# mstebelev/wormhole

Hardware: AMD Instinct MI355X
Metric: examples/sec, DiFacto FM on Criteo-1TB-shaped sparse at 1/2/4/8 MI355X (higher is better)
Workload: dtype fp32; 1 GPU; model=difacto-fm-dim64, global_batch=100000, seq_len=39, parallelism=dp1+kvshard1, minibatch_per_gpu=100000, threshold=100, nnz_per_example=39

## Files before the change

csrc/bind/fm_ops.cc:

```cpp
#include "kv_store.h"
#include "localize_ahead.h"
#include "ps_ops.h"
#include "store_guard.h"

#include <c10/hip/HIPCachingAllocator.h>
#include <c10/hip/HIPGuard.h>

#include <cmath>
#include <cstring>
#include <memory>

#include "host/linear_guard_plan.h"

namespace wh_bind {
namespace {

void check_vstride(int64_t vstride) {
  TORCH_CHECK(vstride == 0 || (vstride >= 4 && vstride <= 256 && (vstride & (vstride - 1)) == 0),
              "vstride must be 0 or 4 * 2^k <= 256, got ", vstride);
}

int loss_flags(int64_t loss, const Tensor& met) {
  return (int)loss | (met.numel() >= 5 ? 256 : 0);
}
// ... 580 lines not shown
 private:
  KVStore* store_;
  std::vector<double> hp_;
  int64_t threshold_;
  bool l1_shrk_;
  int64_t seed_, loss_;
  int vs_ = 0;
  double clip_ = 0, dropout_ = 0;
  bool gnorm_ = false, post_on_ = false, direct_ = false, fused_v_ = false;
  int64_t dim_ = 0;
  StoreGuard guard_;
  LocalizeAhead ahead_;
  std::unique_ptr<HostSplit> timing_{host_split("difacto native step")};
};

}

void bind_fm(py::module_& m) {
  py::class_<LinearStep>(m, "LinearStep")
      .def(py::init<KVStore*, int64_t, double, double, double, double, int64_t, double, bool>(),
           py::arg("store"), py::arg("algo"), py::arg("alpha"), py::arg("beta"), py::arg("l1"),
           py::arg("l2"), py::arg("loss"), py::arg("max_load") = 0.7, py::arg("direct") = true,
           py::keep_alive<1, 2>())
      .def("step", &LinearStep::step, py::arg("keys"), py::arg("offset"), py::arg("val"),
           py::arg("label"), py::arg("train"), py::arg("met"), py::arg("auc_sum"),
           py::arg("next_keys") = py::none(), py::arg("next_offset") = py::none(),
           py::arg("next_val") = py::none(), py::arg("ready") = 0)
      .def("reset", &LinearStep::reset)
      .def("guard_sync", &LinearStep::guard_sync)
      .def_property_readonly("grows", &LinearStep::grows)
      .def_property_readonly("direct", [](const LinearStep& l) { return l.direct(); })
      .def_property("pushes", &LinearStep::pushes, &LinearStep::set_pushes);
  py::class_<DifactoStep>(m, "DifactoStep")
      .def(py::init<KVStore*, std::vector<double>, int64_t, bool, int64_t, int64_t,
                    std::vector<double>, double, bool, bool>(),
           py::arg("store"), py::arg("hp"), py::arg("threshold"), py::arg("l1_shrk"),
           py::arg("seed"), py::arg("loss"), py::arg("post"), py::arg("max_load"),
           py::arg("direct"), py::arg("fused_v") = true, py::keep_alive<1, 2>())
      .def("step", &DifactoStep::step, py::arg("keys"), py::arg("offset"), py::arg("val"),
           py::arg("label"), py::arg("train"), py::arg("data_pass"), py::arg("met"),
           py::arg("auc_sum"), py::arg("step"), py::arg("next_keys") = py::none(),
           py::arg("next_offset") = py::none(), py::arg("next_val") = py::none(),
           py::arg("ready") = 0)
      .def("reset", &DifactoStep::reset)
      .def("guard_sync", &DifactoStep::guard_sync)
      .def_property_readonly("direct", &DifactoStep::direct)
      .def_property_readonly("fused_v", &DifactoStep::fused_v)
      .def_property_readonly("grows", &DifactoStep::grows)
      .def_property_readonly("vgrows", &DifactoStep::vgrows);
  m.def("fm_forward", &fm_forward);
  m.def("set_cu_reserve", [](int64_t n) { wh::fm_set_cu_reserve((int)n); },
        "CUs the persistent FM kernels leave free for concurrent collectives");
  m.def("cu_reserve", []() { return (int64_t)wh::fm_cu_reserve(); });
  m.def("fm_backward", &fm_backward);
  m.def("fm_backward_plan", &fm_backward_plan, py::arg("csc_off"), py::arg("csc_row"),
        py::arg("hdr"), py::arg("vc_rows"), py::arg("nrows"), py::arg("vstride"),
        py::arg("two_pass") = false);
  m.def("fm_backward_run", &fm_backward_run);
  m.def("difacto_open_pull_plan", &difacto_open_pull_plan, py::arg("store"), py::arg("keys"),
        py::arg("insert"), py::arg("cnt"), py::arg("h"), py::arg("threshold"),
        py::arg("l1_shrk"), py::arg("seed"), py::arg("direct"), py::arg("csc_off"),
        py::arg("csc_row"), py::arg("nrows"),
        "(tests) the open with the backward's chunk plan: (slot, hdr, vc, vpos, plan)");
  m.def("fm_backward_plan_totals", &fm_backward_plan_totals, py::arg("plan"),
        py::arg("csc_off"), py::arg("nnz"), py::arg("vstride"),
        "(tests) a backward plan's chunk totals {scalar, V}");
  m.def("fm_grad_post", &fm_grad_post);
  m.def("vstride_for", &vstride_for);
  m.def("spmv_t", &spmv_t, py::arg("csc_off"), py::arg("csc_row"), py::arg("csc_val"),
        py::arg("p"));
}

}
```

csrc/hip/fm.hip:

```cpp
#include "wh_common.h"
#include <string>
#include "kv_device.h"
#include "wh_chunk_plan.h"
#include "wh_kernels.h"
#include "wh_lookback.h"
#include "wh_loss.h"

#include <algorithm>
#include <cstdlib>
#include <type_traits>

namespace wh {
namespace {

constexpr int kThreads = 256;
constexpr int kFwdBlocks = 2048;

template <int G>
struct Shape {
  static constexpr int SUB = 64 / G;
  static constexpr int NI = G;
#ifndef WH_FM_TI
#define WH_FM_TI 4
#endif
// ... 214 lines not shown
  if (k < nuniq) {
    vid = key_vidx(hdr, k);
    const int64_t* off = vid >= 0 ? off_v : off_s;
    c0 = off[k];
    nc = (int32_t)(off[k + 1] - c0);
    b0 = (int32_t)csc_off[k];
    cnt = (int32_t)(csc_off[k + 1] - b0);
  }
  emit_key(out, (int32_t)k, c0, nc, b0, cnt, vid, vid >= 0);
}

constexpr int kPlanPer = 4;
constexpr int kPlanTile = kThreads * kPlanPer;

__global__ __launch_bounds__(kThreads) void k_chunk_plan(int64_t nuniq,
                                                         const int64_t* __restrict__ csc_off,
                                                         const float2* __restrict__ hdr,
                                                         Lookback lb, int ntiles,
                                                         int64_t* off_s_tot, int64_t* off_v_tot,
                                                         ChunkOut out) {
  __shared__ uint32_t shs[16];
  __shared__ int sht;
  const int tile = lb_tile(lb, ntiles, &sht);
  const int64_t k0 = (int64_t)tile * kPlanTile + threadIdx.x * kPlanPer;
  int64_t co[kPlanPer + 1];
#pragma unroll
  for (int r = 0; r <= kPlanPer; ++r) co[r] = k0 + r <= nuniq ? csc_off[k0 + r] : 0;
  int32_t vid[kPlanPer];
#pragma unroll
  for (int r = 0; r < kPlanPer; ++r) vid[r] = k0 + r < nuniq ? key_vidx(hdr, k0 + r) : -1;
  uint32_t c[2] = {0u, 0u};
  uint32_t nc[kPlanPer];
#pragma unroll
  for (int r = 0; r < kPlanPer; ++r) {
    nc[r] = k0 + r < nuniq ? (uint32_t)key_chunks(co[r + 1] - co[r], vid[r] >= 0) : 0u;
    c[vid[r] >= 0 ? 1 : 0] += nc[r];
  }
  uint32_t ex[2], tot[2];
  lb_block_scan<2>(lb, tile, c, ex, tot, shs);
  if (tile == ntiles - 1 && threadIdx.x == 0) {
    *off_s_tot = tot[0];
    *off_v_tot = tot[1];
  }
#pragma unroll
  for (int r = 0; r < kPlanPer; ++r) {
    const int isv = vid[r] >= 0;
    emit_key(out, (int32_t)(k0 + r), isv ? ex[1] : ex[0], (int32_t)nc[r], (int32_t)co[r],
             (int32_t)(co[r + 1] - co[r]), vid[r], isv);
    ex[isv ? 1 : 0] += nc[r];
  }
}

constexpr int kBuckets = 256;
constexpr int kBucketBlocks = 128;
constexpr int kBucketU = 8;

__device__ __forceinline__ int row_bucket(int row, int shift) {
  const int b = row >> shift;
  return b < kBuckets ? b : kBuckets - 1;
}

__global__ __launch_bounds__(kThreads) void k_vchunk_hist(const int64_t* __restrict__ nchunk_p,
                                                          const int4* __restrict__ meta,
                                                          const int32_t* __restrict__ csc_row,
                                                          int shift, int32_t* hist) {
  __shared__ int32_t h[kBuckets];
  for (int i = threadIdx.x; i < kBuckets; i += kThreads) h[i] = 0;
  __syncthreads();
  const int64_t n = *nchunk_p;
  const int64_t per = (n + gridDim.x - 1) / gridDim.x;
  const int64_t c0 = per * blockIdx.x, c1 = c0 + per < n ? c0 + per : n;
  for (int64_t cb = c0 + threadIdx.x; cb < c1; cb += kThreads * kBucketU) {
    int idx[kBucketU], row[kBucketU];
#pragma unroll
    for (int u = 0; u < kBucketU; ++u) {
      const int64_t c = cb + (int64_t)u * kThreads;
      idx[u] = c < c1 ? meta[c].y : -1;
    }
#pragma unroll
    for (int u = 0; u < kBucketU; ++u) row[u] = idx[u] >= 0 ? csc_row[idx[u]] : -1;
#pragma unroll
    for (int u = 0; u < kBucketU; ++u)
      if (row[u] >= 0) atomicAdd(&h[row_bucket(row[u], shift)], 1);
  }
  __syncthreads();
  for (int i = threadIdx.x; i < kBuckets; i += kThreads) hist[blockIdx.x * kBuckets + i] = h[i];
}

constexpr int kScanParts = 4;
constexpr int kScanPer = kBucketBlocks / kScanParts;

__global__ __launch_bounds__(kBuckets * kScanParts) void k_vchunk_scan(int32_t* hist) {
  __shared__ int32_t part[kScanParts][kBuckets];
  __shared__ int32_t excl[kBuckets];
  __shared__ int32_t wtot[kBuckets / 64];
  const int b = threadIdx.x & (kBuckets - 1), q = threadIdx.x / kBuckets;
  int32_t v[kScanPer];
#pragma unroll
  for (int i = 0; i < kScanPer; ++i) v[i] = hist[(q * kScanPer + i) * kBuckets + b];
  int32_t sum = 0;
#pragma unroll
  for (int i = 0; i < kScanPer; ++i) sum += v[i];
  part[q][b] = sum;
  __syncthreads();
  if (q == 0) {
    int32_t t = 0;
#pragma unroll
    for (int r = 0; r < kScanParts; ++r) t += part[r][b];
    const int lane = b & 63;
    int32_t x = t;
#pragma unroll
    for (int o = 1; o < 64; o <<= 1) {
      const int32_t y = __shfl_up(x, o, 64);
      if (lane >= o) x += y;
    }
    if (lane == 63) wtot[b >> 6] = x;
    excl[b] = x - t;
  }
  __syncthreads();
  int32_t base = excl[b];
  for (int w = 0; w < (b >> 6); ++w) base += wtot[w];
  for (int r = 0; r < q; ++r) base += part[r][b];
#pragma unroll
  for (int i = 0; i < kScanPer; ++i) {
    hist[(q * kScanPer + i) * kBuckets + b] = base;
    base += v[i];
  }
}

__global__ __launch_bounds__(kThreads) void k_vchunk_scatter(const int64_t* __restrict__ nchunk_p,
                                                             const int4* __restrict__ meta,
                                                             const int32_t* __restrict__ csc_row,
                                                             int shift,
                                                             const int32_t* __restrict__ hist,
                                                             int4* out) {
  __shared__ int32_t base[kBuckets];
  for (int i = threadIdx.x; i < kBuckets; i += kThreads) base[i] = hist[blockIdx.x * kBuckets + i];
  __syncthreads();
  const int64_t n = *nchunk_p;
  const int64_t per = (n + gridDim.x - 1) / gridDim.x;
  const int64_t c0 = per * blockIdx.x, c1 = c0 + per < n ? c0 + per : n;
  for (int64_t cb = c0 + threadIdx.x; cb < c1; cb += kThreads * kBucketU) {
    int4 m[kBucketU];
    int row[kBucketU];
#pragma unroll
    for (int u = 0; u < kBucketU; ++u) {
      const int64_t c = cb + (int64_t)u * kThreads;
      m[u] = c < c1 ? meta[c] : make_int4(0, -1, 0, 0);
    }
#pragma unroll
    for (int u = 0; u < kBucketU; ++u) row[u] = m[u].y >= 0 ? csc_row[m[u].y] : -1;
#pragma unroll
    for (int u = 0; u < kBucketU; ++u)
      if (row[u] >= 0) out[atomicAdd(&base[row_bucket(row[u], shift)], 1)] = m[u];
  }
}

__global__ __launch_bounds__(kThreads) void k_bwd_scalar(const int64_t* __restrict__ nchunk_p,
                                                         const int32_t* __restrict__ chunk_key,
                                                         const int32_t* __restrict__ chunk_beg,
                                                         const int64_t* __restrict__ csc_off,
                                                         const int32_t* __restrict__ csc_row,
                                                         const float* __restrict__ csc_val,
                                                         const float* __restrict__ dual,
                                                         float* __restrict__ gw_out,
                                                         float* __restrict__ part_gw) {
  const int64_t c = (int64_t)blockIdx.x * kThreads + threadIdx.x;
  if (c >= *nchunk_p) return;
  const int k = chunk_key[c];
  const int kb = (int)csc_off[k], ke = (int)csc_off[k + 1];
  const int b = chunk_beg[c];
  const int e = b + kChunkS < ke ? b + kChunkS : ke;
  float gw = 0.f;
  int p = b;
  for (; p + 3 < e; p += 4) {
    int i[4];
    float x[4];
#pragma unroll
    for (int u = 0; u < 4; ++u) {
      i[u] = csc_row[p + u];
      x[u] = csc_val ? csc_val[p + u] : 1.f;
    }
#pragma unroll
    for (int u = 0; u < 4; ++u) gw += dual[i[u]] * x[u];
  }
  for (; p < e; ++p) gw += dual[csc_row[p]] * (csc_val ? csc_val[p] : 1.f);
  if (ke - kb <= kChunkS) gw_out[k] = gw;
  else if (part_gw) part_gw[c] = gw;
  else atomicAdd(gw_out + k, gw);
}

template <int G, bool FUSED>
__global__ __launch_bounds__(kThreads) void k_bwd_v(const int64_t* __restrict__ nchunk_p,
                                                    const int4* __restrict__ meta,
                                                    const int32_t* __restrict__ csc_row,
                                                    const float* __restrict__ csc_val,
                                                    const float* __restrict__ dual,
                                                    const float* __restrict__ xv,
                                                    const float* __restrict__ vc, int vstride,
                                                    float* __restrict__ gw_out,
                                                    float* __restrict__ gvc,
                                                    float* __restrict__ part_gw,
                                                    float* __restrict__ part_gv, float* fv,
                                                    float* fvg, DifactoHP hp) {
  using S = Shape<G>;
  constexpr bool kSplit = 64 / G >= 4;
  const float* vrows = FUSED ? fv : vc;
  __shared__ int2 stage[kThreads / 64][64];
  int2* st = stage[threadIdx.x >> 6];
  const int lane = threadIdx.x & 63, gl = lane & (G - 1), sub = lane / G;
  const int64_t nch = *nchunk_p, nw = (int64_t)gridDim.x * (kThreads / 64);
  const int64_t w0 =
      __builtin_amdgcn_readfirstlane((int)(((int64_t)blockIdx.x * kThreads + threadIdx.x) >> 6));
  auto get_meta = [&](int64_t c) {
    return c < nch ? meta[c] : make_int4(0, 0, 0, -1);
  };
  auto load_rows = [&](const int4& mt, int& r, float& x) {
    const bool ok = lane < (mt.z & 0xff);
    r = ok ? csc_row[mt.y + lane] : -1;
    x = ok ? (csc_val ? csc_val[mt.y + lane] : 1.f) : 0.f;
  };
  int64_t c = w0;
  int4 mc = get_meta(c), mn = get_meta(c + nw), m2 = get_meta(c + 2 * nw),
       m3 = make_int4(0, 0, 0, -1);
  int rc, rn, r2 = -1;
  float xc, xn, x2 = 0.f;
  load_rows(mc, rc, xc);
  float dc = rc >= 0 ? dual[rc] * xc : 0.f;
  load_rows(mn, rn, xn);
  float dn = 0.f;
  for (; c < nch; c += nw) {
    const int n = mc.z & 0xff;
    const bool multi = (mc.z >> 8) != 0;
    float4 acc = make_float4(0.f, 0.f, 0.f, 0.f);
    float4 v = make_float4(0.f, 0.f, 0.f, 0.f);
    float4 vg = make_float4(0.f, 0.f, 0.f, 0.f);
    stage_pairs<G>(st, lane, rc, dc);
    auto batch = [&](auto tb, int t0) {
      constexpr int TB = decltype(tb)::value;
      float4 a[TB];
      float du[TB];
#pragma unroll
      for (int t = 0; t < TB; ++t) {
        const int2 e = st[sub * S::NI + t0 + t];
        du[t] = __int_as_float(e.y);
        const float* src = e.x >= 0 ? xv + (uint32_t)e.x * (uint32_t)S::VS : kZeroRow;
        a[t] = reinterpret_cast<const float4*>(src)[gl];
      }
      if (t0 == 0) {
        v = reinterpret_cast<const float4*>(vrows + (uint32_t)mc.w * (uint32_t)S::VS)[gl];
        if (FUSED && !multi) {
          if (kSplit) vg.x = fvg[(uint32_t)mc.w * (uint32_t)S::VS + gl * 4 + (sub & 3)];
          else vg = reinterpret_cast<const float4*>(fvg + (uint32_t)mc.w * (uint32_t)S::VS)[gl];
        }
        dn = rn >= 0 ? dual[rn] * xn : 0.f;
        load_rows(m2, r2, x2);
        m3 = get_meta(c + 3 * nw);
      }
#pragma unroll
      for (int t = 0; t < TB; ++t) {
        acc.x += du[t] * a[t].x; acc.y += du[t] * a[t].y;
        acc.z += du[t] * a[t].z; acc.w += du[t] * a[t].w;
      }
    };
    if (n > S::NI * S::SUB / 2) {
      batch(std::integral_constant<int, S::NI>(), 0);
    } else {
#pragma unroll
      for (int t0 = 0; t0 < S::NI; t0 += S::TI) {
        if (t0 * S::SUB >= n) break;
        batch(std::integral_constant<int, S::TI>(), t0);
      }
    }
    if (n == 0) {
      dn = rn >= 0 ? dual[rn] * xn : 0.f;
      load_rows(m2, r2, x2);
      m3 = get_meta(c + 3 * nw);
    }
    const float gw = wave_sum(dc);
    const float xxp = wave_sum(dc * xc);
#pragma unroll
    for (int o = G; o < 64; o <<= 1) {
      acc.x += __shfl_xor(acc.x, o, 64); acc.y += __shfl_xor(acc.y, o, 64);
      acc.z += __shfl_xor(acc.z, o, 64); acc.w += __shfl_xor(acc.w, o, 64);
    }
    if (lane == 0) {
      if (!multi) gw_out[mc.x] = gw;
      else if (part_gw) part_gw[c] = gw;
      else atomicAdd(gw_out + mc.x, gw);
    }
    acc.x -= xxp * v.x; acc.y -= xxp * v.y; acc.z -= xxp * v.z; acc.w -= xxp * v.w;
    if (FUSED && !multi) {
      if (kSplit) {
        const int comp = sub & 3;
        const float a = comp == 0 ? acc.x : comp == 1 ? acc.y : comp == 2 ? acc.z : acc.w;
        float v1 = comp == 0 ? v.x : comp == 1 ? v.y : comp == 2 ? v.z : v.w;
        kvd::adagrad1(v1, vg.x, a, hp);
        if (sub < 4) {
          const uint32_t at = (uint32_t)mc.w * (uint32_t)S::VS + gl * 4 + comp;
          fv[at] = v1;
          fvg[at] = vg.x;
        }
      } else {
        kvd::adagrad4(v, vg, acc, hp);
        if (sub == 0) {
          reinterpret_cast<float4*>(fv + (uint32_t)mc.w * (uint32_t)S::VS)[gl] = v;
          reinterpret_cast<float4*>(fvg + (uint32_t)mc.w * (uint32_t)S::VS)[gl] = vg;
        }
      }
    } else if (!multi || part_gv) {
      float* dst = multi ? part_gv + c * (int64_t)vstride : gvc + (int64_t)mc.w * vstride;
      if (sub == 0) *reinterpret_cast<float4*>(dst + gl * 4) = acc;
    } else {
      float* gv = gvc + (int64_t)mc.w * vstride;
#pragma unroll
      for (int c = 0; c < (S::VS + 63) / 64; ++c) {
        const int d = c * 64 + lane;
        const int src = (d >> 2) & (G - 1);
        const float ax = __shfl(acc.x, src, 64), ay = __shfl(acc.y, src, 64);
        const float az = __shfl(acc.z, src, 64), aw = __shfl(acc.w, src, 64);
        const int comp = d & 3;
        const float a = comp == 0 ? ax : comp == 1 ? ay : comp == 2 ? az : aw;
        if (d < S::VS) atomicAdd(gv + d, a);
      }
    }
    mc = mn; rc = rn; xc = xn; dc = dn;
    mn = m2; rn = r2; xn = x2;
    m2 = m3;
  }
}

__global__ __launch_bounds__(kThreads) void k_bwd_reduce_s(const int64_t* __restrict__ nchunk_p,
                                                           const int32_t* __restrict__ chunk_key,
                                                           const int32_t* __restrict__ chunk_beg,
                                                           const int64_t* __restrict__ csc_off,
                                                           const float* __restrict__ part_gw,
                                                           float* __restrict__ gw_out) {
  const int64_t c = (int64_t)blockIdx.x * kThreads + threadIdx.x;
  if (c >= *nchunk_p) return;
  const int k = chunk_key[c];
  const int64_t kb = csc_off[k], cnt = csc_off[k + 1] - kb;
  if (cnt <= kChunkS || chunk_beg[c] != kb) return;
  const int64_t n = (cnt + kChunkS - 1) / kChunkS;
  float s = 0.f;
  for (int64_t q = 0; q < n; ++q) s += part_gw[c + q];
  gw_out[k] = s;
}

__global__ __launch_bounds__(kThreads) void k_bwd_reduce_v(const int64_t* __restrict__ nchunk_p,
                                                           const int4* __restrict__ meta,
                                                           const int64_t* __restrict__ csc_off,
                                                           const float* __restrict__ part_gw,
                                                           const float* __restrict__ part_gv,
                                                           int vstride, float* __restrict__ gw_out,
                                                           float* __restrict__ gvc) {
  const int lane = threadIdx.x & 63;
  const int64_t c = ((int64_t)blockIdx.x * kThreads + threadIdx.x) >> 6;
  if (c >= *nchunk_p) return;
  const int4 m = meta[c];
  if ((m.z >> 8) == 0 || (int64_t)m.y != csc_off[m.x]) return;
  const int64_t cnt = csc_off[m.x + 1] - m.y;
  const int64_t n = (cnt + kChunkV - 1) / kChunkV;
  float g = 0.f;
  for (int64_t q = 0; q < n; ++q) g += part_gw[c + q];
  for (int d = lane; d < vstride; d += 64) {
    float a = 0.f;
    for (int64_t q = 0; q < n; ++q) a += part_gv[(c + q) * vstride + d];
    gvc[(int64_t)m.w * vstride + d] = a;
  }
  if (lane == 0) gw_out[m.x] = g;
}

__global__ __launch_bounds__(kThreads) void k_grad_post(const int64_t* __restrict__ m_p,
                                                        float* gvc, int vstride, int dim,
                                                        float clip, float dropout, uint64_t seed,
                                                        double* sumsq) {
  __shared__ double sh[kThreads / 64];
  const int64_t total = *m_p * vstride;
  double ss = 0;
  for (int64_t t = (int64_t)blockIdx.x * kThreads + threadIdx.x; t < total;
       t += (int64_t)gridDim.x * kThreads) {
    const int64_t r = t / vstride;
    const int d = (int)(t % vstride);
    if (d >= dim) continue;
    float v = gvc[t];
    if (clip > 0.f) v = fminf(fmaxf(v, -clip), clip);
    if (dropout > 0.f && uhash01(seed, (uint64_t)r, (uint64_t)d) > 1.f - dropout) v = 0.f;
    gvc[t] = v;
    ss += (double)v * v;
  }
  if (sumsq) {
    const double s = block_sum_d(ss, sh);
    if (threadIdx.x == 0) atomicAdd(sumsq, s);
  }
}

__global__ __launch_bounds__(kThreads) void k_grad_scale(const int64_t* __restrict__ m_p,
                                                         float* gvc, int vstride, int dim,
                                                         const double* sumsq) {
  const int64_t t = (int64_t)blockIdx.x * kThreads + threadIdx.x;
  const double n2 = *sumsq;
  if (n2 < 1e-10 || t / vstride >= *m_p || (int)(t % vstride) >= dim) return;
  gvc[t] = (float)(gvc[t] / sqrt(n2));
}

}

template <typename F>
static void dispatch_g(int G, F&& f) {
  switch (G) {
    case 1: f(std::integral_constant<int, 1>()); break;
    case 2: f(std::integral_constant<int, 2>()); break;
    case 4: f(std::integral_constant<int, 4>()); break;
    case 8: f(std::integral_constant<int, 8>()); break;
    case 16: f(std::integral_constant<int, 16>()); break;
    case 32: f(std::integral_constant<int, 32>()); break;
    case 64: f(std::integral_constant<int, 64>()); break;
    default:
      fprintf(stderr, "fm.hip: no kernel for vstride %d (4 * 2^k <= 256 only)\n", 4 * G);
      abort();
  }
}

int64_t fm_fwd_partials() { return 4 * kFwdBlocks; }
int64_t fwd_ticket_words() { return kArriveWords; }

static int g_cu_reserve = 0;

void fm_set_cu_reserve(int cus) { g_cu_reserve = cus < 0 ? 0 : cus; }
int fm_cu_reserve() { return g_cu_reserve; }

static int device_cus() {
  static int cus = 0;
  if (cus == 0) {
    int dev = 0;
    WH_HIP_CHECK(hipGetDevice(&dev));
    WH_HIP_CHECK(hipDeviceGetAttribute(&cus, hipDeviceAttributeMultiprocessorCount, dev));
  }
  return std::max(1, cus - std::min(g_cu_reserve, cus / 2));
}

template <typename K>
static int resident_blocks(K kernel, int cap) {
  const int cus = device_cus();
  int per_cu = 0;
  WH_HIP_CHECK(hipOccupancyMaxActiveBlocksPerMultiprocessor(&per_cu, kernel, kThreads, 0));
  const int n = std::max(1, per_cu) * cus;
  return n < cap ? n : cap;
}

void fm_forward(int64_t nrows, const int64_t* offset, const int32_t* lid, const float* val,
                const float* w_or_hdr, const float* vc, int vstride, const float* label, int loss,
                float* py, float* dual, float* xv, double* met, double* part,
                unsigned int* ticket, hipStream_t s) {
  if (nrows <= 0) return;
  const int acc5 = (loss >> 8) & 1;
  loss &= 0xff;
  if (vstride == 0) {
    constexpr int G = 8;
    const int nblk = grid_for(nrows * G, kThreads, kFwdBlocks);
    hipLaunchKernelGGL(k_lin_fwd<G>, dim3(nblk), dim3(kThreads), 0, s, nrows, offset, lid, val,
                       w_or_hdr, 1, label, loss, py, dual, part, met, ticket, acc5);
    return;
  }
  const float2* hdr = reinterpret_cast<const float2*>(w_or_hdr);
  dispatch_g(vstride / 4, [&](auto g) {
    constexpr int G = decltype(g)::value;
    const int nblk =
        grid_for(nrows * 64, kThreads, resident_blocks(k_fm_fwd<G>, kFwdBlocks));
    hipLaunchKernelGGL(k_fm_fwd<G>, dim3(nblk), dim3(kThreads), 0, s, nrows, offset, lid, val,
                       hdr, vc, vstride, label, loss, py, dual, xv, part, met, ticket, acc5);
  });
}

void lin_forward_strided(int64_t nrows, const int64_t* offset, const int32_t* lid,
                         const float* val, const float* w, int wstride, const float* label,
                         int loss, float* py, float* dual, double* met, double* part,
                         unsigned int* ticket, hipStream_t s) {
  if (nrows <= 0) return;
  const int acc5 = (loss >> 8) & 1;
  loss &= 0xff;
  constexpr int G = 8;
  const int nblk = grid_for(nrows * G, kThreads, kFwdBlocks);
  hipLaunchKernelGGL(k_lin_fwd<G>, dim3(nblk), dim3(kThreads), 0, s, nrows, offset, lid, val, w,
                     wstride, label, loss, py, dual, part, met, ticket, acc5);
}

static int64_t scalar_cap(int64_t nuniq, int64_t nnz) { return nuniq + nnz / kChunkS + 1; }
static int64_t v_cap(int64_t nuniq, int64_t nnz) { return nuniq + nnz / kChunkV + 1; }

static int bucket_shift(int64_t nrows) {
  int shift = 0;
  while ((((nrows - 1) >> shift) >= kBuckets)) ++shift;
  return shift;
}

int64_t fm_bwd_layout(int64_t nuniq, int64_t nnz, int vstride, bool deterministic,
                      FmBwdLayout* out) {
  int64_t at = 0;
  auto carve = [&](int64_t bytes) {
    const int64_t o = at;
    at += (bytes + 255) / 256 * 256;
    return o;
  };
  const int64_t cap_s = scalar_cap(nuniq, nnz), cap_v = vstride > 0 ? v_cap(nuniq, nnz) : 0;
  FmBwdLayout l;
  l.key_s = carve(cap_s * 4);
  l.beg_s = carve(cap_s * 4);
  l.meta_v = carve(2 * cap_v * 16);
  l.hist = carve(vstride > 0 ? (int64_t)kBuckets * kBucketBlocks * 4 : 0);
  l.det_s = carve(deterministic ? cap_s * 4 : 0);
  l.det_vw = carve(deterministic ? cap_v * 4 : 0);
  l.det_v = carve(deterministic ? cap_v * vstride * 4 : 0);
  l.off = carve(2 * (nuniq + 1) * 8);
  l.cnt = carve(2 * nuniq * 8);
  l.scan_tmp = carve(scan_tmp_elems(nuniq) * 8);
  if (out) *out = l;
  return at;
}

FmBwdPlanDst fm_bwd_plan_dst(const FmBwdProblem& p, void* scratch) {
  FmBwdLayout l;
  fm_bwd_layout(p.nuniq, p.nnz, p.vstride, p.deterministic, &l);
  char* base = static_cast<char*>(scratch);
  int64_t* off_s = reinterpret_cast<int64_t*>(base + l.off);
  return {p.csc_off, reinterpret_cast<int32_t*>(base + l.key_s),
          reinterpret_cast<int32_t*>(base + l.beg_s), base + l.meta_v, p.gw, p.gvc, p.vstride,
          off_s + p.nuniq, off_s + p.nuniq + 1 + p.nuniq};
}

void fm_backward(const FmBwdProblem& p, void* scratch, const Lookback* lb, hipStream_t s,
                 FmBwdPhase phase) {
  const int64_t nuniq = p.nuniq;
  if (nuniq <= 0) return;
  const int vstride = p.vstride;
  const float2* hdr = vstride > 0 ? reinterpret_cast<const float2*>(p.hdr) : nullptr;
  FmBwdLayout l;
  fm_bwd_layout(nuniq, p.nnz, vstride, p.deterministic, &l);
  char* base = static_cast<char*>(scratch);
  int32_t* key_s = reinterpret_cast<int32_t*>(base + l.key_s);
  int32_t* beg_s = reinterpret_cast<int32_t*>(base + l.beg_s);
  int4* meta_v = reinterpret_cast<int4*>(base + l.meta_v);
  int64_t* off_s = reinterpret_cast<int64_t*>(base + l.off);
  int64_t* off_v = off_s + nuniq + 1;
  const int64_t cap_s = scalar_cap(nuniq, p.nnz), cap_v = v_cap(nuniq, p.nnz);
  const bool bucket =
      hdr && !p.deterministic && p.nrows * (int64_t)vstride * 4 > ((int64_t)2 << 20);
  int4* meta_sorted = bucket ? meta_v + cap_v : meta_v;
  if (phase == FmBwdPhase::kAll || phase == FmBwdPhase::kPlan) {
    const ChunkOut out = {key_s, beg_s, meta_v, p.gw, p.gvc, vstride};
    const int64_t ntiles = (nuniq + kPlanTile - 1) / kPlanTile;
    if (lb && ntiles <= kLbMaxTiles) {
      hipLaunchKernelGGL(k_chunk_plan, dim3((unsigned)ntiles), dim3(kThreads), 0, s, nuniq,
                         p.csc_off, hdr, *lb, (int)ntiles, off_s + nuniq, off_v + nuniq, out);
    } else {
      int64_t* cnt_s = reinterpret_cast<int64_t*>(base + l.cnt);
      int64_t* cnt_v = cnt_s + nuniq;
      int64_t* scan_tmp = reinterpret_cast<int64_t*>(base + l.scan_tmp);
      const dim3 grid(grid_for(nuniq, kThreads));
      hipLaunchKernelGGL(k_chunk_count, grid, dim3(kThreads), 0, s, nuniq, p.csc_off, hdr, cnt_s,
                         cnt_v);
      scan_i64(cnt_s, off_s, nuniq, scan_tmp, s);
      if (hdr) scan_i64(cnt_v, off_v, nuniq, scan_tmp, s);
      hipLaunchKernelGGL(k_chunk_fill, grid, dim3(kThreads), 0, s, nuniq, p.csc_off, off_s, off_v,
                         hdr, out);
    }
  }
  if (phase != FmBwdPhase::kRun && bucket) {
    int32_t* hist = reinterpret_cast<int32_t*>(base + l.hist);
    const int shift = bucket_shift(std::max<int64_t>(p.nrows, 1));
    hipLaunchKernelGGL(k_vchunk_hist, dim3(kBucketBlocks), dim3(kThreads), 0, s, off_v + nuniq,
                       meta_v, p.csc_row, shift, hist);
    hipLaunchKernelGGL(k_vchunk_scan, dim3(1), dim3(kBuckets * kScanParts), 0, s, hist);
    hipLaunchKernelGGL(k_vchunk_scatter, dim3(kBucketBlocks), dim3(kThreads), 0, s,
                       off_v + nuniq, meta_v, p.csc_row, shift, hist, meta_sorted);
  }
  if (phase == FmBwdPhase::kPlan || phase == FmBwdPhase::kBucket) return;
  const bool det = p.deterministic;
  float* pgs = det ? reinterpret_cast<float*>(base + l.det_s) : nullptr;
  float* pgv_w = det ? reinterpret_cast<float*>(base + l.det_vw) : nullptr;
  float* pgv = det ? reinterpret_cast<float*>(base + l.det_v) : nullptr;
  hipLaunchKernelGGL(k_bwd_scalar, dim3(grid_for(cap_s, kThreads)), dim3(kThreads), 0, s,
                     off_s + nuniq, key_s, beg_s, p.csc_off, p.csc_row, p.csc_val, p.dual, p.gw,
                     pgs);
  if (det)
    hipLaunchKernelGGL(k_bwd_reduce_s, dim3(grid_for(cap_s, kThreads)), dim3(kThreads), 0, s,
                       off_s + nuniq, key_s, beg_s, p.csc_off, pgs, p.gw);
  if (!hdr) return;
  dispatch_g(vstride / 4, [&](auto g) {
    constexpr int G = decltype(g)::value;
    auto run = [&](auto kernel, const float* vc) {
      const int64_t vblk = std::min<int64_t>((cap_v + 3) / 4, resident_blocks(kernel, 2048));
      hipLaunchKernelGGL(kernel, dim3((unsigned)vblk), dim3(kThreads), 0, s, off_v + nuniq,
                         meta_sorted, p.csc_row, p.csc_val, p.dual, p.xv, vc, vstride, p.gw,
                         p.gvc, pgv_w, pgv, p.fuse_v, p.fuse_vg, p.fuse_hp);
    };
    if (p.fuse_v && p.fuse_v != p.vc) {
      fprintf(stderr, "fm.hip: the fused update needs vc to be the V slab itself\n");
      abort();
    }
    if (p.fuse_v) run(k_bwd_v<G, true>, nullptr);
    else run(k_bwd_v<G, false>, p.vc);
  });
  if (det)
    hipLaunchKernelGGL(k_bwd_reduce_v, dim3(grid_for(cap_v * 64, kThreads)), dim3(kThreads), 0, s,
                       off_v + nuniq, meta_v, p.csc_off, pgv_w, pgv, vstride, p.gw, p.gvc);
}

void fm_grad_post(const int64_t* m, int64_t m_cap, float* gvc, int vstride, int dim, float clip,
                  float dropout, uint64_t seed, double* sumsq, hipStream_t s) {
  if (m_cap <= 0 || vstride == 0) return;
  hipLaunchKernelGGL(k_grad_post, dim3(grid_for(m_cap * vstride, kThreads, 1024)), dim3(kThreads),
                     0, s, m, gvc, vstride, dim, clip, dropout, seed, sumsq);
}

void fm_grad_scale(const int64_t* m, int64_t m_cap, float* gvc, int vstride, int dim,
                   const double* sumsq, hipStream_t s) {
  if (m_cap <= 0 || vstride == 0) return;
  hipLaunchKernelGGL(k_grad_scale, dim3(grid_for(m_cap * vstride, kThreads)), dim3(kThreads), 0,
                     s, m, gvc, vstride, dim, sumsq);
}

}
```

csrc/hip/wh_kernels.h:

```cpp
#pragma once
#include <hip/hip_runtime.h>
#include <stdint.h>

namespace wh {

int64_t scan_tmp_elems(int64_t n);
void scan_i32(const int32_t* in, int64_t* out, int64_t n, int64_t* tmp, hipStream_t s);
void scan_i64(const int64_t* in, int64_t* out, int64_t n, int64_t* tmp, hipStream_t s);
constexpr int kLbMaxTiles = 1 << 16;
constexpr int kLbChannels = 3;
struct Lookback {
  unsigned long long* gran;
  unsigned int* ticket;
  unsigned int* err;
  unsigned int epoch;
};
int64_t lookback_ws_words();
Lookback lookback_bind(void* ws);

void loc_insert(const uint64_t* keys, int64_t nnz, uint64_t* tkeys, int64_t tsize,
                int32_t* slot_of, int64_t* overflow, hipStream_t s);
void key_mod(uint64_t* keys, int64_t n, uint64_t m, hipStream_t s);
int64_t loc_owner_blocks(int64_t tsize);
void loc_owner_count(const uint64_t* tkeys, int64_t tsize, int nshard, int64_t* blkcnt,
// ... 108 lines not shown
                        const Lookback& lb, float* hdr, int64_t* vpos, float* vc, hipStream_t s);
struct FmBwdPlanDst;
bool difacto_open_pull(const KVTable& t, const uint64_t* keys, int64_t n, const int32_t* cnt,
                       DifactoHP hp, int insert, const Lookback& lb, int32_t* slot, float* hdr,
                       int64_t* vpos, float* vc, hipStream_t s,
                       const FmBwdPlanDst* plan = nullptr);
bool vidx_renumber_fused(float* hdr, int64_t n, const Lookback& lb, int64_t* count,
                         hipStream_t s);

struct PsPrep {
  uint32_t* chain = nullptr;
  int64_t n = 0;
  int32_t* vbase = nullptr;
};
bool ps_open(const KVTable& t, const uint64_t* keys, const int32_t* rec, int64_t n, int use_cnt,
             DifactoHP hp, int insert, int chains, uint32_t epoch, int32_t* vbase,
             const int64_t* segS, const int64_t* segHS, int P, const Lookback& lb, int32_t* slot,
             float* w_out, int64_t* vpos, uint32_t* chain, uint8_t* head, float* rbuf,
             int64_t* vcnt, hipStream_t s, int prepped = 0);
bool ps_push(const KVTable& t, const int32_t* slot, const int64_t* vpos, const uint32_t* chain,
             const uint8_t* head, int64_t n, const int64_t* segS, const int64_t* segHS, int P,
             const float* gbuf, DifactoHP hp, hipStream_t s, PsPrep prep = PsPrep());
void ps_records(const uint64_t* uniq, const int32_t* ucnt, int64_t U, int32_t* rec,
                hipStream_t s);
bool ps_c0(const int64_t* owner_cnt, const int64_t* vcnt, int S, int P, int64_t flag,
           int64_t* send, int64_t* payload, hipStream_t s, int loop = 0);
bool ps_push_linear(const KVTable& t, const int32_t* slot, const uint32_t* chain,
                    const uint8_t* head, int64_t n, const int64_t* segS, int P, const float* g,
                    LinearHP hp, double t0, hipStream_t s, PsPrep prep = PsPrep());
bool ps_unpack(const float* rbuf, int64_t U, int vstride, const int64_t* segS,
               const int64_t* segHS, const int64_t* vrecv, int P, float* hdr, int64_t* rows_total,
               hipStream_t s);
bool ps_pack_gw(const float* gw, int64_t U, int vstride, const int64_t* segS,
                const int64_t* segHS, const int64_t* vrecv, int P, float* gbuf, hipStream_t s);

int64_t fm_fwd_partials();
int64_t fwd_ticket_words();
void lin_forward_strided(int64_t nrows, const int64_t* offset, const int32_t* lid,
                         const float* val, const float* w, int wstride, const float* label,
                         int loss, float* py, float* dual, double* met, double* part,
                         unsigned int* ticket, hipStream_t s);
int ld_rows_per_tile(int64_t nnz, int64_t nrows);
int ld_tile_table(int64_t nnz);
void ld_touch(const KVTable& t, const uint64_t* keys, const int64_t* off, int64_t nrows,
              int64_t nnz, int R, uint32_t stamp, int insert, int32_t* lid, int32_t* tlist,
              unsigned int* tcnt, int32_t* ovf, unsigned int* ovf_cnt, hipStream_t s);
void ld_backward(const int32_t* lid, const float* val, const int64_t* off, int64_t nrows,
                 int64_t nnz, int R, const float* dual, float* grad, hipStream_t s);
void ld_push(const KVTable& t, int64_t ntiles, int T, const int32_t* tlist,
             const unsigned int* tcnt, const int32_t* ovf, unsigned int* ovf_cnt, float* grad,
             LinearHP hp, hipStream_t s);
void fm_set_cu_reserve(int cus);
int fm_cu_reserve();
void fm_forward(int64_t nrows, const int64_t* offset, const int32_t* lid, const float* val,
                const float* w_or_hdr, const float* vc, int vstride, const float* label, int loss,
                float* py, float* dual, float* xv, double* met, double* part,
                unsigned int* ticket, hipStream_t s);
struct FmBwdProblem {
  int64_t nuniq, nnz, nrows;
  const int64_t* csc_off;
  const int32_t* csc_row;
  const float* csc_val;
  const float *dual, *xv;
  const float *hdr, *vc;
  int vstride;
  float *gw, *gvc;
  bool deterministic;
  float* fuse_v = nullptr;
  float* fuse_vg = nullptr;
  DifactoHP fuse_hp = {};
};
constexpr int kChunkV = 64;
enum class FmBwdPhase { kAll, kPlan, kRun, kBucket, kBucketRun };
struct FmBwdLayout {
  int64_t key_s, beg_s;
  int64_t meta_v;
  int64_t hist;
  int64_t det_s, det_vw, det_v;
  int64_t off;
  int64_t cnt, scan_tmp;
};
int64_t fm_bwd_layout(int64_t nuniq, int64_t nnz, int vstride, bool deterministic,
                      FmBwdLayout* out = nullptr);
struct FmBwdPlanDst {
  const int64_t* csc_off;
  int32_t *key_s, *beg_s;
  void* meta_v;
  float *gw, *gvc;
  int vstride;
  int64_t *tot_s, *tot_v;
};
FmBwdPlanDst fm_bwd_plan_dst(const FmBwdProblem& p, void* scratch);
void fm_backward(const FmBwdProblem& p, void* scratch, const Lookback* lb, hipStream_t s,
                 FmBwdPhase phase);
void fm_grad_post(const int64_t* m, int64_t m_cap, float* gvc, int vstride, int dim, float clip,
                  float dropout, uint64_t seed, double* sumsq, hipStream_t s);
void fm_grad_scale(const int64_t* m, int64_t m_cap, float* gvc, int vstride, int dim,
                   const double* sumsq, hipStream_t s);

void spmv(int64_t nrows, const int64_t* off, const int32_t* col, const float* val, const float* x,
          float* y, hipStream_t s);
size_t auc_sort_tmp_bytes(int64_t n);
void sort_by_score(const float* py, const float* label, int64_t n, float* py_sorted,
                   float* label_sorted, void* tmp, size_t tmp_bytes, hipStream_t s);
void auc_from_sorted(const float* label_sorted, int64_t n, double* out, int64_t* tmp_i64,
                     hipStream_t s);
// ... 209 lines not shown
```

Measured before the change: 141.5 million examples/s.

## Pack small single-chunk keys into lane groups in FM V backward

The backward V kernel can now process several small keys (at most TI nonzeros, one chunk) per wavefront, assigning one G-lane group to each key instead of one whole wavefront per key. The bucket sort gains a second digit so that small chunks are grouped together, which makes whole-wave packable groups more likely, and the scan kernel is generalised to the larger digit count. The change also staggers wave assignment across blocks and reworks the prefetch pipeline. It targets wasted lanes on the many rare low-count keys in Criteo-like data, at the cost of more complex control flow and a wider histogram. Packing is on by default and can be turned off with an environment variable or a Python setter.

```diff
diff --git a/csrc/bind/fm_ops.cc b/csrc/bind/fm_ops.cc
--- a/csrc/bind/fm_ops.cc
+++ b/csrc/bind/fm_ops.cc
@@ -656,6 +656,9 @@
   m.def("set_cu_reserve", [](int64_t n) { wh::fm_set_cu_reserve((int)n); },
         "CUs the persistent FM kernels leave free for concurrent collectives");
   m.def("cu_reserve", []() { return (int64_t)wh::fm_cu_reserve(); });
+  m.def("set_fm_bwd_pack", [](bool on) { wh::fm_set_bwd_pack(on); },
+        "FM backward: pack small single-chunk keys, one lane group per key (default on)");
+  m.def("fm_bwd_pack", []() { return wh::fm_bwd_pack(); });
   m.def("fm_backward", &fm_backward);
   m.def("fm_backward_plan", &fm_backward_plan, py::arg("csc_off"), py::arg("csc_row"),
         py::arg("hdr"), py::arg("vc_rows"), py::arg("nrows"), py::arg("vstride"),
diff --git a/csrc/hip/fm.hip b/csrc/hip/fm.hip
--- a/csrc/hip/fm.hip
+++ b/csrc/hip/fm.hip
@@ -290,6 +290,7 @@
 }
 
 constexpr int kBuckets = 256;
+constexpr int kDigits = 2 * kBuckets;
 constexpr int kBucketBlocks = 128;
 constexpr int kBucketU = 8;
 
@@ -298,53 +299,68 @@
   return b < kBuckets ? b : kBuckets - 1;
 }
 
+__device__ __forceinline__ bool small_chunk(int z, int small_n) { return z >= 1 && z <= small_n; }
+
+template <int D>
+__device__ __forceinline__ int chunk_digit(int row, int shift, int z, int small_n) {
+  const int b = row_bucket(row, shift);
+  return D == kBuckets ? b : b * 2 + (small_chunk(z, small_n) ? 0 : 1);
+}
+
+template <int D>
 __global__ __launch_bounds__(kThreads) void k_vchunk_hist(const int64_t* __restrict__ nchunk_p,
                                                           const int4* __restrict__ meta,
                                                           const int32_t* __restrict__ csc_row,
-                                                          int shift, int32_t* hist) {
-  __shared__ int32_t h[kBuckets];
-  for (int i = threadIdx.x; i < kBuckets; i += kThreads) h[i] = 0;
+                                                          int shift, int small_n, int32_t* hist) {
+  __shared__ int32_t h[D];
+  for (int i = threadIdx.x; i < D; i += kThreads) h[i] = 0;
   __syncthreads();
   const int64_t n = *nchunk_p;
   const int64_t per = (n + gridDim.x - 1) / gridDim.x;
   const int64_t c0 = per * blockIdx.x, c1 = c0 + per < n ? c0 + per : n;
   for (int64_t cb = c0 + threadIdx.x; cb < c1; cb += kThreads * kBucketU) {
-    int idx[kBucketU], row[kBucketU];
+    int idx[kBucketU], z[kBucketU], row[kBucketU];
 #pragma unroll
     for (int u = 0; u < kBucketU; ++u) {
       const int64_t c = cb + (int64_t)u * kThreads;
       idx[u] = c < c1 ? meta[c].y : -1;
+      z[u] = D != kBuckets && c < c1 ? meta[c].z : 0;
     }
 #pragma unroll
     for (int u = 0; u < kBucketU; ++u) row[u] = idx[u] >= 0 ? csc_row[idx[u]] : -1;
 #pragma unroll
     for (int u = 0; u < kBucketU; ++u)
-      if (row[u] >= 0) atomicAdd(&h[row_bucket(row[u], shift)], 1);
+      if (row[u] >= 0) atomicAdd(&h[chunk_digit<D>(row[u], shift, z[u], small_n)], 1);
   }
   __syncthreads();
-  for (int i = threadIdx.x; i < kBuckets; i += kThreads) hist[blockIdx.x * kBuckets + i] = h[i];
-}
-
-constexpr int kScanParts = 4;
-constexpr int kScanPer = kBucketBlocks / kScanParts;
-
-__global__ __launch_bounds__(kBuckets * kScanParts) void k_vchunk_scan(int32_t* hist) {
-  __shared__ int32_t part[kScanParts][kBuckets];
-  __shared__ int32_t excl[kBuckets];
-  __shared__ int32_t wtot[kBuckets / 64];
-  const int b = threadIdx.x & (kBuckets - 1), q = threadIdx.x / kBuckets;
-  int32_t v[kScanPer];
-#pragma unroll
-  for (int i = 0; i < kScanPer; ++i) v[i] = hist[(q * kScanPer + i) * kBuckets + b];
+  for (int i = threadIdx.x; i < D; i += kThreads) hist[blockIdx.x * D + i] = h[i];
+}
+
+constexpr int kScanThreads = 1024;
+
+template <int D>
+__global__ __launch_bounds__(kScanThreads) void k_vchunk_scan(int32_t* hist) {
+  constexpr int kParts = kScanThreads / D, kPer = kBucketBlocks / kParts;
+  constexpr int kKeep = kPer <= 32 ? kPer : 32;
+  __shared__ int32_t part[kParts][D];
+  __shared__ int32_t excl[D];
+  __shared__ int32_t wtot[D / 64];
+  const int b = threadIdx.x & (D - 1), q = threadIdx.x / D;
+  int32_t v[kKeep];
   int32_t sum = 0;
 #pragma unroll
-  for (int i = 0; i < kScanPer; ++i) sum += v[i];
+  for (int i0 = 0; i0 < kPer; i0 += kKeep) {
+#pragma unroll
+    for (int i = 0; i < kKeep; ++i) v[i] = hist[(q * kPer + i0 + i) * D + b];
+#pragma unroll
+    for (int i = 0; i < kKeep; ++i) sum += v[i];
+  }
   part[q][b] = sum;
   __syncthreads();
   if (q == 0) {
     int32_t t = 0;
 #pragma unroll
-    for (int r = 0; r < kScanParts; ++r) t += part[r][b];
+    for (int r = 0; r < kParts; ++r) t += part[r][b];
     const int lane = b & 63;
     int32_t x = t;
 #pragma unroll
@@ -360,20 +376,28 @@
   for (int w = 0; w < (b >> 6); ++w) base += wtot[w];
   for (int r = 0; r < q; ++r) base += part[r][b];
 #pragma unroll
-  for (int i = 0; i < kScanPer; ++i) {
-    hist[(q * kScanPer + i) * kBuckets + b] = base;
-    base += v[i];
-  }
-}
-
+  for (int i0 = 0; i0 < kPer; i0 += kKeep) {
+    if (kPer > kKeep) {
+#pragma unroll
+      for (int i = 0; i < kKeep; ++i) v[i] = hist[(q * kPer + i0 + i) * D + b];
+    }
+#pragma unroll
+    for (int i = 0; i < kKeep; ++i) {
+      hist[(q * kPer + i0 + i) * D + b] = base;
+      base += v[i];
+    }
+  }
+}
+
+template <int D>
 __global__ __launch_bounds__(kThreads) void k_vchunk_scatter(const int64_t* __restrict__ nchunk_p,
                                                              const int4* __restrict__ meta,
                                                              const int32_t* __restrict__ csc_row,
-                                                             int shift,
+                                                             int shift, int small_n,
                                                              const int32_t* __restrict__ hist,
                                                              int4* out) {
-  __shared__ int32_t base[kBuckets];
-  for (int i = threadIdx.x; i < kBuckets; i += kThreads) base[i] = hist[blockIdx.x * kBuckets + i];
+  __shared__ int32_t base[D];
+  for (int i = threadIdx.x; i < D; i += kThreads) base[i] = hist[blockIdx.x * D + i];
   __syncthreads();
   const int64_t n = *nchunk_p;
   const int64_t per = (n + gridDim.x - 1) / gridDim.x;
@@ -390,7 +414,8 @@
     for (int u = 0; u < kBucketU; ++u) row[u] = m[u].y >= 0 ? csc_row[m[u].y] : -1;
 #pragma unroll
     for (int u = 0; u < kBucketU; ++u)
-      if (row[u] >= 0) out[atomicAdd(&base[row_bucket(row[u], shift)], 1)] = m[u];
+      if (row[u] >= 0)
+        out[atomicAdd(&base[chunk_digit<D>(row[u], shift, m[u].z, small_n)], 1)] = m[u];
   }
 }
 
@@ -440,7 +465,7 @@
                                                     float* __restrict__ gvc,
                                                     float* __restrict__ part_gw,
                                                     float* __restrict__ part_gv, float* fv,
-                                                    float* fvg, DifactoHP hp) {
+                                                    float* fvg, DifactoHP hp, int pack) {
   using S = Shape<G>;
   constexpr bool kSplit = 64 / G >= 4;
   const float* vrows = FUSED ? fv : vc;
@@ -448,26 +473,135 @@
   int2* st = stage[threadIdx.x >> 6];
   const int lane = threadIdx.x & 63, gl = lane & (G - 1), sub = lane / G;
   const int64_t nch = *nchunk_p, nw = (int64_t)gridDim.x * (kThreads / 64);
-  const int64_t w0 =
-      __builtin_amdgcn_readfirstlane((int)(((int64_t)blockIdx.x * kThreads + threadIdx.x) >> 6));
-  auto get_meta = [&](int64_t c) {
-    return c < nch ? meta[c] : make_int4(0, 0, 0, -1);
+  const bool can_pack = pack != 0 && S::SUB > 1;
+  const int gs = can_pack ? S::SUB : 1;
+  const int64_t ngrp = (nch + gs - 1) / gs;
+  const int wv = __builtin_amdgcn_readfirstlane((int)(threadIdx.x >> 6));
+  const int64_t w0 = (gridDim.x & 7) == 0
+                         ? (int64_t)(blockIdx.x & 7) * (nw / 8) + (blockIdx.x >> 3) * (kThreads / 64) + wv
+                         : (int64_t)blockIdx.x * (kThreads / 64) + wv;
+  const int4 kNone = make_int4(0, 0, 0, -1);
+  const int64_t e_last = nch > 0 ? nch - 1 : 0;
+  auto get_group = [&](int64_t g) {
+    const int64_t e = g * gs + (can_pack ? sub : 0);
+    const int4 m = meta[e < e_last ? e : e_last];
+    return e < nch ? m : kNone;
   };
-  auto load_rows = [&](const int4& mt, int& r, float& x) {
-    const bool ok = lane < (mt.z & 0xff);
-    r = ok ? csc_row[mt.y + lane] : -1;
-    x = ok ? (csc_val ? csc_val[mt.y + lane] : 1.f) : 0.f;
+  int64_t gq = w0;
+  int jq = 0;
+  int4 mg = get_group(gq);
+  bool load_mg = false;
+  auto plan_item = [&](int4& im, int& vid, bool& pk, int64_t& e, int& at) {
+    const bool ok = gq < ngrp;
+    pk = can_pack && __ballot(small_chunk(mg.z, S::TI)) == ~0ull;
+    e = gq * gs + jq;
+    load_mg = true;
+    int beg, n, i;
+    if (pk) {
+      vid = mg.w;
+      beg = mg.y;
+      n = mg.z;
+      i = gl;
+    } else {
+      const int src = jq * G;
+      im = make_int4(__builtin_amdgcn_readlane(mg.x, src), __builtin_amdgcn_readlane(mg.y, src),
+                     __builtin_amdgcn_readlane(mg.z, src), __builtin_amdgcn_readlane(mg.w, src));
+      beg = im.y;
+      n = im.z & 0xff;
+      i = lane;
+      ++jq;
+      load_mg = jq >= gs || gq * gs + jq >= nch;
+    }
+    at = i < n ? beg + i : -1;
+    if (load_mg) {
+      gq += nw;
+      jq = 0;
+    }
+    return ok;
   };
-  int64_t c = w0;
-  int4 mc = get_meta(c), mn = get_meta(c + nw), m2 = get_meta(c + 2 * nw),
-       m3 = make_int4(0, 0, 0, -1);
-  int rc, rn, r2 = -1;
+  auto issue_item = [&](int at, int& r, float& x) {
+    r = at >= 0 ? csc_row[at] : -1;
+    x = at >= 0 ? (csc_val ? csc_val[at] : 1.f) : 0.f;
+    if (load_mg) mg = get_group(gq);
+  };
+  int4 mc = kNone, mn = kNone, m2 = kNone;
+  int vic = -1, vin = -1, vi2 = -1;
+  bool pc, pn, p2 = false;
+  int64_t ec, en, e2 = 0;
+  int rc, rn, r2 = -1, at2 = -1;
   float xc, xn, x2 = 0.f;
-  load_rows(mc, rc, xc);
-  float dc = rc >= 0 ? dual[rc] * xc : 0.f;
-  load_rows(mn, rn, xn);
+  bool okc = plan_item(mc, vic, pc, ec, at2);
+  issue_item(at2, rc, xc);
+  float dc = (rc >= 0 ? dual[rc] : 0.f) * xc;
+  bool okn = plan_item(mn, vin, pn, en, at2), ok2 = false;
+  issue_item(at2, rn, xn);
   float dn = 0.f;
-  for (; c < nch; c += nw) {
+  auto prefetch = [&]() {
+    dn = rn >= 0 ? dual[rn] : 0.f;
+    issue_item(at2, r2, x2);
+  };
+  while (okc) {
+    ok2 = plan_item(m2, vi2, p2, e2, at2);
+    if (pc) {
+      if (gl < S::TI) st[sub * S::NI + gl] = make_int2(rc, __float_as_int(dc));
+      __builtin_amdgcn_fence(__ATOMIC_RELEASE, "wavefront");
+      __builtin_amdgcn_wave_barrier();
+      __builtin_amdgcn_fence(__ATOMIC_ACQUIRE, "wavefront");
+      float4 a[S::TI];
+      float du[S::TI];
+#pragma unroll
+      for (int t = 0; t < S::TI; ++t) {
+        const int2 e = st[sub * S::NI + t];
+        du[t] = __int_as_float(e.y);
+        const float* src = e.x >= 0 ? xv + (uint32_t)e.x * (uint32_t)S::VS : kZeroRow;
+        a[t] = reinterpret_cast<const float4*>(src)[gl];
+      }
+      const uint32_t vat = (uint32_t)vic * (uint32_t)S::VS;
+      float4 v = reinterpret_cast<const float4*>(vrows + vat)[gl];
+      float4 vg = make_float4(0.f, 0.f, 0.f, 0.f);
+      if (FUSED) vg = reinterpret_cast<const float4*>(fvg + vat)[gl];
+      const int key = meta[ec + sub].x;
+      prefetch();
+      constexpr int W = S::SUB < S::TI ? S::SUB : S::TI;
+      float4 q[W];
+#pragma unroll
+      for (int j = 0; j < W; ++j) q[j] = make_float4(0.f, 0.f, 0.f, 0.f);
+#pragma unroll
+      for (int t = 0; t < S::TI; ++t) {
+        float4& p = q[t % S::SUB];
+        p.x += du[t] * a[t].x; p.y += du[t] * a[t].y;
+        p.z += du[t] * a[t].z; p.w += du[t] * a[t].w;
+      }
+#pragma unroll
+      for (int o = 1; o < W; o <<= 1) {
+#pragma unroll
+        for (int j = 0; j + o < W; j += 2 * o) {
+          q[j].x += q[j + o].x; q[j].y += q[j + o].y;
+          q[j].z += q[j + o].z; q[j].w += q[j + o].w;
+        }
+      }
+      float4 acc = q[0];
+#pragma unroll
+      for (int o = W; o < S::SUB; o <<= 1) {
+        acc.x += 0.f; acc.y += 0.f; acc.z += 0.f; acc.w += 0.f;
+      }
+      float gw = dc + 0.f, xx = dc * xc + 0.f;
+#pragma unroll
+      for (int o = S::TI / 2; o > 0; o >>= 1) {
+        gw += __shfl_xor(gw, o, 64);
+        xx += __shfl_xor(xx, o, 64);
+      }
+      const float xxp = __shfl(xx, lane & ~(G - 1), 64);
+      if (gl == 0) gw_out[key] = gw;
+      acc.x -= xxp * v.x; acc.y -= xxp * v.y; acc.z -= xxp * v.z; acc.w -= xxp * v.w;
+      if (FUSED) {
+        kvd::adagrad4(v, vg, acc, hp);
+        reinterpret_cast<float4*>(fv + vat)[gl] = v;
+        reinterpret_cast<float4*>(fvg + vat)[gl] = vg;
+      } else {
+        *reinterpret_cast<float4*>(gvc + (int64_t)vic * vstride + gl * 4) = acc;
+      }
+    } else {
     const int n = mc.z & 0xff;
     const bool multi = (mc.z >> 8) != 0;
     float4 acc = make_float4(0.f, 0.f, 0.f, 0.f);
@@ -491,9 +625,7 @@
           if (kSplit) vg.x = fvg[(uint32_t)mc.w * (uint32_t)S::VS + gl * 4 + (sub & 3)];
           else vg = reinterpret_cast<const float4*>(fvg + (uint32_t)mc.w * (uint32_t)S::VS)[gl];
         }
-        dn = rn >= 0 ? dual[rn] * xn : 0.f;
-        load_rows(m2, r2, x2);
-        m3 = get_meta(c + 3 * nw);
+        prefetch();
       }
 #pragma unroll
       for (int t = 0; t < TB; ++t) {
@@ -510,11 +642,7 @@
         batch(std::integral_constant<int, S::TI>(), t0);
       }
     }
-    if (n == 0) {
-      dn = rn >= 0 ? dual[rn] * xn : 0.f;
-      load_rows(m2, r2, x2);
-      m3 = get_meta(c + 3 * nw);
-    }
+    if (n == 0) prefetch();
     const float gw = wave_sum(dc);
     const float xxp = wave_sum(dc * xc);
 #pragma unroll
@@ -524,7 +652,7 @@
     }
     if (lane == 0) {
       if (!multi) gw_out[mc.x] = gw;
-      else if (part_gw) part_gw[c] = gw;
+      else if (part_gw) part_gw[ec] = gw;
       else atomicAdd(gw_out + mc.x, gw);
     }
     acc.x -= xxp * v.x; acc.y -= xxp * v.y; acc.z -= xxp * v.z; acc.w -= xxp * v.w;
@@ -547,7 +675,7 @@
         }
       }
     } else if (!multi || part_gv) {
-      float* dst = multi ? part_gv + c * (int64_t)vstride : gvc + (int64_t)mc.w * vstride;
+      float* dst = multi ? part_gv + ec * (int64_t)vstride : gvc + (int64_t)mc.w * vstride;
       if (sub == 0) *reinterpret_cast<float4*>(dst + gl * 4) = acc;
     } else {
       float* gv = gvc + (int64_t)mc.w * vstride;
@@ -562,9 +690,9 @@
         if (d < S::VS) atomicAdd(gv + d, a);
       }
     }
-    mc = mn; rc = rn; xc = xn; dc = dn;
-    mn = m2; rn = r2; xn = x2;
-    m2 = m3;
+    }
+    mc = mn; vic = vin; pc = pn; okc = okn; ec = en; rc = rn; xc = xn; dc = dn * xn;
+    mn = m2; vin = vi2; pn = p2; okn = ok2; en = e2; rn = r2; xn = x2;
   }
 }
 
@@ -668,6 +796,17 @@
 void fm_set_cu_reserve(int cus) { g_cu_reserve = cus < 0 ? 0 : cus; }
 int fm_cu_reserve() { return g_cu_reserve; }
 
+static int g_bwd_pack = -1;
+
+void fm_set_bwd_pack(bool on) { g_bwd_pack = on ? 1 : 0; }
+bool fm_bwd_pack() {
+  if (g_bwd_pack < 0) {
+    const char* e = std::getenv("WH_FM_BWD_PACK");
+    g_bwd_pack = !(e && std::string(e) == "0");
+  }
+  return g_bwd_pack == 1;
+}
+
 static int device_cus() {
   static int cus = 0;
   if (cus == 0) {
@@ -746,7 +885,7 @@
   l.key_s = carve(cap_s * 4);
   l.beg_s = carve(cap_s * 4);
   l.meta_v = carve(2 * cap_v * 16);
-  l.hist = carve(vstride > 0 ? (int64_t)kBuckets * kBucketBlocks * 4 : 0);
+  l.hist = carve(vstride > 0 ? (int64_t)kDigits * kBucketBlocks * 4 : 0);
   l.det_s = carve(deterministic ? cap_s * 4 : 0);
   l.det_vw = carve(deterministic ? cap_v * 4 : 0);
   l.det_v = carve(deterministic ? cap_v * vstride * 4 : 0);
@@ -785,6 +924,7 @@
   const bool bucket =
       hdr && !p.deterministic && p.nrows * (int64_t)vstride * 4 > ((int64_t)2 << 20);
   int4* meta_sorted = bucket ? meta_v + cap_v : meta_v;
+  const bool pack = fm_bwd_pack();
   if (phase == FmBwdPhase::kAll || phase == FmBwdPhase::kPlan) {
     const ChunkOut out = {key_s, beg_s, meta_v, p.gw, p.gvc, vstride};
     const int64_t ntiles = (nuniq + kPlanTile - 1) / kPlanTile;
@@ -807,11 +947,18 @@
   if (phase != FmBwdPhase::kRun && bucket) {
     int32_t* hist = reinterpret_cast<int32_t*>(base + l.hist);
     const int shift = bucket_shift(std::max<int64_t>(p.nrows, 1));
-    hipLaunchKernelGGL(k_vchunk_hist, dim3(kBucketBlocks), dim3(kThreads), 0, s, off_v + nuniq,
-                       meta_v, p.csc_row, shift, hist);
-    hipLaunchKernelGGL(k_vchunk_scan, dim3(1), dim3(kBuckets * kScanParts), 0, s, hist);
-    hipLaunchKernelGGL(k_vchunk_scatter, dim3(kBucketBlocks), dim3(kThreads), 0, s,
-                       off_v + nuniq, meta_v, p.csc_row, shift, hist, meta_sorted);
+    const int G = vstride / 4;
+    const int small_n = pack && G < 64 ? std::min(G, WH_FM_TI) : 0;
+    auto sort = [&](auto d) {
+      constexpr int D = decltype(d)::value;
+      hipLaunchKernelGGL(k_vchunk_hist<D>, dim3(kBucketBlocks), dim3(kThreads), 0, s,
+                         off_v + nuniq, meta_v, p.csc_row, shift, small_n, hist);
+      hipLaunchKernelGGL(k_vchunk_scan<D>, dim3(1), dim3(kScanThreads), 0, s, hist);
+      hipLaunchKernelGGL(k_vchunk_scatter<D>, dim3(kBucketBlocks), dim3(kThreads), 0, s,
+                         off_v + nuniq, meta_v, p.csc_row, shift, small_n, hist, meta_sorted);
+    };
+    if (small_n > 0) sort(std::integral_constant<int, kDigits>());
+    else sort(std::integral_constant<int, kBuckets>());
   }
   if (phase == FmBwdPhase::kPlan || phase == FmBwdPhase::kBucket) return;
   const bool det = p.deterministic;
@@ -831,7 +978,7 @@
       const int64_t vblk = std::min<int64_t>((cap_v + 3) / 4, resident_blocks(kernel, 2048));
       hipLaunchKernelGGL(kernel, dim3((unsigned)vblk), dim3(kThreads), 0, s, off_v + nuniq,
                          meta_sorted, p.csc_row, p.csc_val, p.dual, p.xv, vc, vstride, p.gw,
-                         p.gvc, pgv_w, pgv, p.fuse_v, p.fuse_vg, p.fuse_hp);
+                         p.gvc, pgv_w, pgv, p.fuse_v, p.fuse_vg, p.fuse_hp, pack ? 1 : 0);
     };
     if (p.fuse_v && p.fuse_v != p.vc) {
       fprintf(stderr, "fm.hip: the fused update needs vc to be the V slab itself\n");
diff --git a/csrc/hip/wh_kernels.h b/csrc/hip/wh_kernels.h
--- a/csrc/hip/wh_kernels.h
+++ b/csrc/hip/wh_kernels.h
@@ -184,6 +184,8 @@
              LinearHP hp, hipStream_t s);
 void fm_set_cu_reserve(int cus);
 int fm_cu_reserve();
+void fm_set_bwd_pack(bool on);
+bool fm_bwd_pack();
 void fm_forward(int64_t nrows, const int64_t* offset, const int32_t* lid, const float* val,
                 const float* w_or_hdr, const float* vc, int vstride, const float* label, int loss,
                 float* py, float* dual, float* xv, double* met, double* part,
```

Measured after the change: 158.9 million examples/s (median of 6 runs). +12.3%, better.
